# okian/kofft

Measured on AMD Instinct MI355X. Metric: batched 4096-pt c32 FFT throughput, GPoints/s (achieved HBM GB/s: roofline.achieved), higher is better.
Workload: dtype f32

## Files before the change

include/kofft_hip.h:

```cpp
#ifndef KOFFT_HIP_H
#define KOFFT_HIP_H

#include <stddef.h>

#ifdef __cplusplus
extern "C" {
#endif

#define KOFFT_OK 0
#define KOFFT_ERR_EMPTY_INPUT 1
#define KOFFT_ERR_NON_POWER_OF_TWO_NO_STD 2
#define KOFFT_ERR_MISMATCHED_LENGTHS 3
#define KOFFT_ERR_INVALID_STRIDE 4
#define KOFFT_ERR_INVALID_HOP_SIZE 5
#define KOFFT_ERR_INVALID_VALUE 6
#define KOFFT_ERR_HIP (-1)
#define KOFFT_ERR_UNSUPPORTED (-2)
#define KOFFT_ERR_NULL (-3)
#define KOFFT_ERR_ALLOC (-4)
#define KOFFT_ERR_RCCL (-5)

typedef struct kofft_hip_ctx kofft_hip_ctx;

const char *kofft_hip_strerror(int status);
// ... 58 lines not shown
int kofft_hip_rfft_f64_dev(kofft_hip_ctx *ctx, const double *d_in, double *d_out,
                           const double *d_window, size_t n, size_t batch);
int kofft_hip_irfft_f64(kofft_hip_ctx *ctx, const double *in, double *out, size_t n, size_t batch);
int kofft_hip_irfft_f64_dev(kofft_hip_ctx *ctx, const double *d_in, double *d_out, size_t n,
                            size_t batch);

int kofft_hip_dct2_f32(kofft_hip_ctx *ctx, const float *in, float *out, size_t n, size_t batch);
int kofft_hip_dct2_f32_dev(kofft_hip_ctx *ctx, const float *d_in, float *d_out, size_t n, size_t batch);
int kofft_hip_set_dct_fused(kofft_hip_ctx *ctx, int on);

int kofft_hip_hilbert_f32(kofft_hip_ctx *ctx, const float *in, float *out, size_t n, size_t batch);
int kofft_hip_hilbert_f32_dev(kofft_hip_ctx *ctx, const float *d_in, float *d_out, size_t n, size_t batch);
int kofft_hip_set_hilbert_fused(kofft_hip_ctx *ctx, int on);

int kofft_hip_cepstrum_f32(kofft_hip_ctx *ctx, const float *in, float *out, size_t n, size_t batch);
int kofft_hip_cepstrum_f32_dev(kofft_hip_ctx *ctx, const float *d_in, float *d_out, size_t n, size_t batch);
int kofft_hip_set_cepstrum_fused(kofft_hip_ctx *ctx, int on);

int kofft_hip_dct_direct_f32(kofft_hip_ctx *ctx, int type, const float *in, float *out, size_t n, size_t batch);
int kofft_hip_dct_direct_f32_dev(kofft_hip_ctx *ctx, int type, const float *d_in, float *d_out, size_t n, size_t batch);
int kofft_hip_dst_direct_f32(kofft_hip_ctx *ctx, int type, const float *in, float *out, size_t n, size_t batch);
int kofft_hip_dst_direct_f32_dev(kofft_hip_ctx *ctx, int type, const float *d_in, float *d_out, size_t n, size_t batch);
int kofft_hip_set_direct_tiled(kofft_hip_ctx *ctx, int on);
int kofft_hip_dct_direct_table_f32(int type, size_t n, float *C);
int kofft_hip_dst_direct_table_f32(int type, size_t n, float *C);
int kofft_hip_dst_planner_table_f32(int type, size_t n, float *out);
int kofft_hip_dst_planner_table_f64(int type, size_t n, double *out);

int kofft_hip_czt_f32(kofft_hip_ctx *ctx, const float *in, float *out, size_t n, size_t m, float wr, float wi, float ar, float ai,
                      size_t batch);
int kofft_hip_dev_czt_f32(kofft_hip_ctx *ctx, const float *d_in, float *d_out, size_t n, size_t m, float wr, float wi, float ar, float ai,
                          size_t batch);
int kofft_hip_goertzel_f32(kofft_hip_ctx *ctx, const float *in, float *out, size_t n, size_t batch, float sample_rate,
                           const float *target_freqs, size_t nfreq);
int kofft_hip_dev_goertzel_f32(kofft_hip_ctx *ctx, const float *d_in, float *d_out, size_t n, size_t batch, float sample_rate,
                               const float *target_freqs, size_t nfreq);
int kofft_hip_set_czt_route(kofft_hip_ctx *ctx, int mode);
int kofft_hip_czt_table_f32(size_t n, size_t m, float wr, float wi, float ar, float ai, float *C);
int kofft_hip_goertzel_coeff_f32(size_t n, float sample_rate, const float *target_freqs, size_t nfreq, float *coeff);

#define KOFFT_WAVELET_HAAR 0
#define KOFFT_WAVELET_DB2 1
#define KOFFT_WAVELET_DB4 2
#define KOFFT_WAVELET_SYM4 3
#define KOFFT_WAVELET_COIF1 4
int kofft_hip_dwt_f32(kofft_hip_ctx *ctx, int wavelet, const float *in, float *approx, float *detail, size_t len, size_t batch);
// ... 110 lines not shown
```

kofft_amd/_lib.py:

```python
from __future__ import annotations

import ctypes as C
import os
import re
from pathlib import Path

_PKG = Path(__file__).resolve().parent
LIB_PATH = _PKG / "lib" / "libkofft_hip.so"
HEADER_PATH = _PKG.parent / "include" / "kofft_hip.h"


class LibraryMissing(RuntimeError):
    pass


_c_f = C.POINTER(C.c_float)
_c_d = C.POINTER(C.c_double)
_sz = C.c_size_t
_ctx = C.c_void_p

SIGNATURES = {
    "kofft_hip_strerror": (C.c_char_p, [C.c_int]),
    "kofft_hip_last_error": (C.c_char_p, [_ctx]),
    "kofft_hip_version": (C.c_char_p, []),
# ... 33 lines not shown
    "kofft_hip_fft_c64_strided": (C.c_int, [_ctx, C.c_void_p, _sz, _sz, _sz, C.c_int]),
    "kofft_hip_rfft_f32": (C.c_int, [_ctx, C.c_void_p, C.c_void_p, C.c_void_p, _sz, _sz]),
    "kofft_hip_rfft_f32_dev": (C.c_int, [_ctx, C.c_void_p, C.c_void_p, C.c_void_p, _sz, _sz]),
    "kofft_hip_irfft_f32": (C.c_int, [_ctx, C.c_void_p, C.c_void_p, _sz, _sz]),
    "kofft_hip_irfft_f32_dev": (C.c_int, [_ctx, C.c_void_p, C.c_void_p, _sz, _sz]),
    "kofft_hip_rfft_f64": (C.c_int, [_ctx, C.c_void_p, C.c_void_p, C.c_void_p, _sz, _sz]),
    "kofft_hip_rfft_f64_dev": (C.c_int, [_ctx, C.c_void_p, C.c_void_p, C.c_void_p, _sz, _sz]),
    "kofft_hip_irfft_f64": (C.c_int, [_ctx, C.c_void_p, C.c_void_p, _sz, _sz]),
    "kofft_hip_irfft_f64_dev": (C.c_int, [_ctx, C.c_void_p, C.c_void_p, _sz, _sz]),
    "kofft_hip_dct2_f32": (C.c_int, [_ctx, C.c_void_p, C.c_void_p, _sz, _sz]),
    "kofft_hip_dct2_f32_dev": (C.c_int, [_ctx, C.c_void_p, C.c_void_p, _sz, _sz]),
    "kofft_hip_set_dct_fused": (C.c_int, [_ctx, C.c_int]),
    "kofft_hip_hilbert_f32": (C.c_int, [_ctx, C.c_void_p, C.c_void_p, _sz, _sz]),
    "kofft_hip_hilbert_f32_dev": (C.c_int, [_ctx, C.c_void_p, C.c_void_p, _sz, _sz]),
    "kofft_hip_set_hilbert_fused": (C.c_int, [_ctx, C.c_int]),
    "kofft_hip_cepstrum_f32": (C.c_int, [_ctx, C.c_void_p, C.c_void_p, _sz, _sz]),
    "kofft_hip_cepstrum_f32_dev": (C.c_int, [_ctx, C.c_void_p, C.c_void_p, _sz, _sz]),
    "kofft_hip_set_cepstrum_fused": (C.c_int, [_ctx, C.c_int]),
    "kofft_hip_dct_direct_f32": (C.c_int, [_ctx, C.c_int, C.c_void_p, C.c_void_p, _sz, _sz]),
    "kofft_hip_dct_direct_f32_dev": (C.c_int, [_ctx, C.c_int, C.c_void_p, C.c_void_p, _sz, _sz]),
    "kofft_hip_dst_direct_f32": (C.c_int, [_ctx, C.c_int, C.c_void_p, C.c_void_p, _sz, _sz]),
    "kofft_hip_dst_direct_f32_dev": (C.c_int, [_ctx, C.c_int, C.c_void_p, C.c_void_p, _sz, _sz]),
    "kofft_hip_set_direct_tiled": (C.c_int, [_ctx, C.c_int]),
    "kofft_hip_dct_direct_table_f32": (C.c_int, [C.c_int, _sz, C.c_void_p]),
    "kofft_hip_dst_direct_table_f32": (C.c_int, [C.c_int, _sz, C.c_void_p]),
    "kofft_hip_dst_planner_table_f32": (C.c_int, [C.c_int, _sz, C.c_void_p]),
    "kofft_hip_dst_planner_table_f64": (C.c_int, [C.c_int, _sz, C.c_void_p]),
    "kofft_hip_czt_f32": (C.c_int, [_ctx, C.c_void_p, C.c_void_p, _sz, _sz, C.c_float, C.c_float, C.c_float, C.c_float, _sz]),
    "kofft_hip_dev_czt_f32": (C.c_int, [_ctx, C.c_void_p, C.c_void_p, _sz, _sz, C.c_float, C.c_float, C.c_float, C.c_float, _sz]),
    "kofft_hip_goertzel_f32": (C.c_int, [_ctx, C.c_void_p, C.c_void_p, _sz, _sz, C.c_float, C.c_void_p, _sz]),
    "kofft_hip_dev_goertzel_f32": (C.c_int, [_ctx, C.c_void_p, C.c_void_p, _sz, _sz, C.c_float, C.c_void_p, _sz]),
    "kofft_hip_set_czt_route": (C.c_int, [_ctx, C.c_int]),
    "kofft_hip_czt_table_f32": (C.c_int, [_sz, _sz, C.c_float, C.c_float, C.c_float, C.c_float, C.c_void_p]),
    "kofft_hip_goertzel_coeff_f32": (C.c_int, [_sz, C.c_float, C.c_void_p, _sz, C.c_void_p]),
    "kofft_hip_dwt_f32": (C.c_int, [_ctx, C.c_int, C.c_void_p, C.c_void_p, C.c_void_p, _sz, _sz]),
    "kofft_hip_dwt_f32_dev": (C.c_int, [_ctx, C.c_int, C.c_void_p, C.c_void_p, C.c_void_p, _sz, _sz]),
    "kofft_hip_idwt_f32": (C.c_int, [_ctx, C.c_int, C.c_void_p, C.c_void_p, C.c_void_p, _sz, _sz]),
    "kofft_hip_idwt_f32_dev": (C.c_int, [_ctx, C.c_int, C.c_void_p, C.c_void_p, C.c_void_p, _sz, _sz]),
    "kofft_hip_dwt_multi_f32": (C.c_int, [_ctx, C.c_int, C.c_void_p, C.c_void_p, C.c_void_p, _sz, _sz, _sz]),
    "kofft_hip_dwt_multi_f32_dev": (C.c_int, [_ctx, C.c_int, C.c_void_p, C.c_void_p, C.c_void_p, _sz, _sz, _sz]),
    "kofft_hip_idwt_multi_f32": (C.c_int, [_ctx, C.c_int, C.c_void_p, C.c_void_p, C.c_void_p, C.c_void_p, _sz, _sz, _sz]),
    "kofft_hip_idwt_multi_f32_dev": (C.c_int, [_ctx, C.c_int, C.c_void_p, C.c_void_p, C.c_void_p, C.c_void_p, _sz, _sz, _sz]),
    "kofft_hip_set_wavelet_fused": (C.c_int, [_ctx, C.c_int]),
    "kofft_hip_dwt_multi_lengths": (C.c_int, [_sz, _sz, C.c_void_p]),
    "kofft_hip_wavelet_taps_f32": (C.c_int, [C.c_int, C.c_int, C.c_void_p, C.c_void_p]),
    "kofft_hip_stft_f32": (C.c_int, [_ctx, C.c_void_p, _sz, C.c_void_p, _sz, _sz, C.c_void_p, _sz]),
# ... 78 lines not shown
```

kofft_amd/api.py:

```python
from __future__ import annotations

import ctypes as C
import os
import enum
from typing import Optional, Sequence

import numpy as np

from . import _lib


class FftError(Exception):

    EmptyInput = 1
    NonPowerOfTwoNoStd = 2
    MismatchedLengths = 3
    InvalidStride = 4
    InvalidHopSize = 5
    InvalidValue = 6
    _names = {1: "EmptyInput", 2: "NonPowerOfTwoNoStd", 3: "MismatchedLengths", 4: "InvalidStride",
              5: "InvalidHopSize", 6: "InvalidValue"}

    def __init__(self, code: int):
        self.code = int(code)
# ... 495 lines not shown
        self._check(getattr(self._lib, f"kofft_hip_{family}_direct_f32")(self._ctx, int(type), _ptr(a), _ptr(out), a.shape[1], a.shape[0]))
        return out

    def dct_direct_batch(self, x: np.ndarray, type: int) -> np.ndarray:
        return self._direct_batch("dct", x, type)

    def dst_direct_batch(self, x: np.ndarray, type: int) -> np.ndarray:
        return self._direct_batch("dst", x, type)

    def _direct_dev(self, family: str, type: int, d_in: int, d_out: int, n: int, batch: int) -> None:
        if min(int(n), int(batch)) < 0:
            raise ValueError("n and batch are usize in the reference: they cannot be negative")
        self._check(getattr(self._lib, f"kofft_hip_{family}_direct_f32_dev")(self._ctx, int(type), C.c_void_p(d_in), C.c_void_p(d_out),
                                                                             int(n), int(batch)))

    def dct_direct_dev(self, type: int, d_in: int, d_out: int, n: int, batch: int) -> None:
        self._direct_dev("dct", type, d_in, d_out, n, batch)

    def dst_direct_dev(self, type: int, d_in: int, d_out: int, n: int, batch: int) -> None:
        self._direct_dev("dst", type, d_in, d_out, n, batch)

    def set_direct_tiled(self, on: bool) -> None:
        self._check(self._lib.kofft_hip_set_direct_tiled(self._ctx, int(bool(on))))

    def set_czt_route(self, mode: int) -> None:
        self._check(self._lib.kofft_hip_set_czt_route(self._ctx, int(mode)))

    def _spectral_in(self, x, what: str):
        if self.dtype != np.float32:
            raise TypeError(f"{what} is f32-only, like the reference ({what}.rs)")
        dev = hasattr(x, "data_ptr") and hasattr(x, "is_cuda")
        if dev:
            import torch

            if not x.is_cuda or x.dtype != torch.float32:
                raise TypeError(f"{what}: a torch input must be a float32 tensor on the device")
            a = x.contiguous()
        else:
            a = np.ascontiguousarray(x, np.float32)
        if a.ndim not in (1, 2):
            raise TypeError(f"{what} expects a 1-D signal or a 2-D [batch, n] array")
        return (a.reshape(1, -1) if a.ndim == 1 else a), a.ndim == 1, dev

    def czt(self, x, m: int, w, a):
        rows, one, dev = self._spectral_in(x, "czt")
        if int(m) < 0:
# ... 1019 lines not shown
```

kofft_amd/csrc/fft_persist.hip.h:

```cpp
#pragma once

#include "fft_wg.hip.h"

namespace kofft {

template <typename T, int L, int S0, int Q>
__device__ __forceinline__ void load_pass_twiddles(cpx<T> *twr, const int k, const cpx<T> *__restrict__ tw)
{
#pragma unroll
    for (int t = 0; t < Q; ++t) {
#pragma unroll
        for (int h = 0; h < (1 << t); ++h) {
            const int idx = (k << (L - 1 - S0 - t)) + (bitrev(h, t) << (L - 1 - t));
            twr[(1 << t) - 1 + h] = tw[idx];
        }
    }
}

template <typename T, int Q>
__device__ __forceinline__ void reg_pass_r(cpx<T> *v, const cpx<T> *twr)
{
#pragma unroll
    for (int t = 0; t < Q; ++t) {
        const int pos = Q - 1 - t;
// ... 73 lines not shown
}

template <bool WAVE>
__device__ __forceinline__ void exchange_sync()
{
    if constexpr (WAVE) {
        __builtin_amdgcn_fence(__ATOMIC_RELEASE, "wavefront");
        __builtin_amdgcn_wave_barrier();
        __builtin_amdgcn_fence(__ATOMIC_ACQUIRE, "wavefront");
    } else {
        __syncthreads();
    }
}

template <class CFG, class = void>
struct persist_depth { static constexpr int value = 1; };
template <class CFG>
struct persist_depth<CFG, decltype((void)CFG::DEPTH)> { static constexpr int value = CFG::DEPTH; };

template <class CFG, class = void>
struct persist_tw_global { static constexpr bool value = false; };
template <class CFG>
struct persist_tw_global<CFG, decltype((void)CFG::kTwGlobal)> { static constexpr bool value = CFG::kTwGlobal; };

template <typename T, int L, int RL, int EPI, class IO, class CFG>
struct PersistState {
    static constexpr int R = 1 << RL;
    static constexpr int NP = (L + RL - 1) / RL;
    static constexpr bool TWG = persist_tw_global<CFG>::value;
    static constexpr bool TW1_REG = !TWG && !(NP == 2 && CFG::kTwLastInLds);
    static constexpr bool TW2_REG = !TWG && NP >= 3 && !(CFG::kTwLastInLds && NP == 3);
    static constexpr bool TW3_REG = !TWG && NP >= 4 && !CFG::kTwLastInLds;
    cpx<T> tw1[TW1_REG ? R - 1 : 1], tw2[TW2_REG ? R - 1 : 1], tw3[TW3_REG ? R - 1 : 1];
    typename IO::Inv inv[CFG::kInvInLds ? 1 : R];
    const typename IO::Inv *inv_lds;
    const cpx<T> *tw_lds;
    const cpx<T> *rt_lds;
    int g1, g2, g3, sc;
};

template <class IO, int TPT, bool PAIR = io_pairs_in_wave<IO>::value>
struct persist_raw {
    using type = typename IO::Raw;
    static constexpr int extra = 0;
    static constexpr bool pair = false, pair_lds = false;
};
template <class IO, int TPT>
struct persist_raw<IO, TPT, true> {
    using type = typename IO::RawPair;
    static constexpr int extra = 1;
    static constexpr bool pair = TPT <= 64, pair_lds = TPT > 64;
};

struct NoAcc {};
template <class IO, bool HAS = io_has_acc<IO>::value>
struct persist_acc { using type = NoAcc; };
template <class IO>
struct persist_acc<IO, true> { using type = typename IO::Acc; };

#ifndef KOFFT_TWG_TOP_PART
#define KOFFT_TWG_TOP_PART -1
#endif
__host__ __device__ constexpr bool persist_twg_top_part(int L) { return KOFFT_TWG_TOP_PART < 0 ? L <= 12 : KOFFT_TWG_TOP_PART != 0; }
struct NoPrefetchParts {
    __device__ __forceinline__ void operator()(int) const {}
};
template <typename T, int L, int RL, int EPI, class CFG, class IO, class Parts = NoPrefetchParts>
__device__ __forceinline__ void persist_transform(const typename persist_raw<IO, ((1 << L) >> RL)>::type *raw,
                                                  const PersistState<T, L, RL, EPI, IO, CFG> &st,
                                                  const IO &io, const cpx<T> *__restrict__ tw, cpx<T> *buf0, cpx<T> *buf1,
                                                  const size_t xf0, const int cnt, const int sub, const int tau,
                                                  typename persist_acc<IO>::type &acc, const Parts &part = Parts{})
{
    constexpr int NBUF = CFG::NBUF;
    constexpr int N = 1 << L;
    constexpr int R = 1 << RL;
    constexpr int TPT = N / R;
    constexpr int NP = (L + RL - 1) / RL;
    constexpr bool WAVE = (TPT <= 64);
    const size_t xf = xf0 + sub;
    const bool active = sub < cnt;
    using LastG = PassGeom<L, RL, NP - 1>;
    using FirstG = PassGeom<L, RL, 0>;

    cpx<T> cur[R];
    constexpr int GRP = TPT >= 64 ? 1 : 64 / TPT;
    if constexpr (persist_raw<IO, TPT>::pair) {
        static_assert(CFG::kInvInLds, "paired input: the table entries come from the LDS copy");
        io.template finish_pairs<R, TPT>(raw, tau, cur, [&](int u) { return (st.inv_lds + tau)[FirstG::in_index(0, u)]; });
    } else if constexpr (persist_raw<IO, TPT>::pair_lds) {
        static_assert(CFG::kInvInLds && NBUF == 1 && !WAVE, "paired input through the exchange buffer");
        exchange_sync<WAVE>();
#pragma unroll
        for (int u = 0; u < R; ++u) buf0[tau + u * TPT] = raw[u];
        if (tau == 0) buf0[N] = raw[R];
// ... 26 lines not shown
    if (NBUF == 1) exchange_sync<WAVE>();
    persist_lds_scatter<T, L, RL, 0>(cur, buf0, st.sc);
    exchange_sync<WAVE>();
    persist_lds_gather<T, L, RL, 1>(cur, buf0, st.g1);
    using St = PersistState<T, L, RL, EPI, IO, CFG>;
    int tau_tw = tau;
    if constexpr (St::TWG) asm volatile("" : "+v"(tau_tw));
    auto pass_tw_global = [&](auto pass) {
        constexpr int P = decltype(pass)::value;
        using Gp = PassGeom<L, RL, P>;
        cpx<T> twr[Gp::G * ((1 << Gp::Q) - 1)];
        persist_load_tw<T, L, RL, P>(twr, tau_tw, tw);
        __builtin_amdgcn_sched_barrier(0);
        part(P - (persist_twg_top_part(L) ? 0 : 1));
        __builtin_amdgcn_sched_barrier(0);
        persist_compute<T, L, RL, P>(cur, twr);
    };
    if constexpr (St::TWG) pass_tw_global(std::integral_constant<int, 1>{});
    else if constexpr (NP == 2 && CFG::kTwLastInLds) wg_compute<T, L, RL, 1>(cur, io, st.tw_lds, xf, tau);
    else persist_compute<T, L, RL, 1>(cur, st.tw1);
    if constexpr (NP >= 3) {
        if (NBUF == 1) exchange_sync<WAVE>();
        persist_lds_scatter<T, L, RL, 1>(cur, buf1, st.sc);
        exchange_sync<WAVE>();
        persist_lds_gather<T, L, RL, 2>(cur, buf1, st.g2);
        if constexpr (St::TWG) pass_tw_global(std::integral_constant<int, 2>{});
        else if constexpr (NP == 3 && CFG::kTwLastInLds) wg_compute<T, L, RL, 2>(cur, io, st.tw_lds, xf, tau);
        else persist_compute<T, L, RL, 2>(cur, st.tw2);
    }
    if constexpr (NP == 4) {
        exchange_sync<WAVE>();
        persist_lds_scatter<T, L, RL, 2>(cur, buf0, st.sc);
        exchange_sync<WAVE>();
        persist_lds_gather<T, L, RL, 3>(cur, buf0, st.g3);
        if constexpr (St::TWG) pass_tw_global(std::integral_constant<int, 3>{});
        else if constexpr (CFG::kTwLastInLds) wg_compute<T, L, RL, 3>(cur, io, st.tw_lds, xf, tau);
        else persist_compute<T, L, RL, 3>(cur, st.tw3);
    }

    if constexpr (EPI == EPI_RFFT) {
        static_assert(L <= 12 || !CFG::kInvInLds, "rfft epilogue: a staged window does not fit next to an 8192-point exchange buffer and the post-pass table");
        cpx<T> *ybuf = (NP == 3) ? buf0 : buf1;
        if (NBUF == 1) exchange_sync<WAVE>();
        {
            cpx<T> *p = ybuf + tau;
#pragma unroll
            for (int u = 0; u < R; ++u) p[LastG::out_index(0, u)] = cur[u];
// ... 126 lines not shown
            for (int i = tid; i < N; i += BLOCK) inv_lds[i] = io.invariant(i);
        } else {
#pragma unroll
            for (int u = 0; u < R; ++u) st.inv[u] = io.invariant(FirstG::in_index(0, u) + tau);
        }
        if constexpr (EPI == EPI_RFFT) {
            for (int i = tid; i < N; i += BLOCK) rt_lds[i] = io.rtab[i];
        }
        if constexpr (CFG::kTwLastInLds) {
            for (int i = tid; i < N / 2; i += BLOCK) tw_lds[i] = tw[i];
        }
        st.inv_lds = inv_lds;
        st.rt_lds = rt_lds;
        st.tw_lds = tw_lds;
        if constexpr (CFG::kInvInLds || CFG::kTwLastInLds || EPI == EPI_RFFT) __syncthreads();
    }
    st.g1 = lds_pad(PassGeom<L, RL, 1>::in_index(tau, 0));
    st.g2 = (NP >= 3) ? lds_pad(PassGeom<L, RL, (NP >= 3 ? 2 : 1)>::in_index(tau, 0)) : 0;
    st.g3 = (NP == 4) ? lds_pad(PassGeom<L, RL, NP - 1>::in_index(tau, 0)) : 0;
    st.sc = lds_pad(tau);

    const size_t step = (size_t)gridDim.x * XPB;
    size_t base = (size_t)blockIdx.x * XPB;
    if (base >= batch) return;

    constexpr int DEPTH = persist_depth<CFG>::value;
    static_assert(DEPTH == 1 || DEPTH == 2, "prefetch distance");
    Raw ra[RS], rb[RS];
    const int in_lane_bytes = tau * IO::kRawBytes;
    const int in_row_off = (G == 1) ? 0 : sub * (int)io.in_slot_bytes();
    auto group_cnt = [&](size_t b) -> int {
        const size_t first = b + wslot;
        return first >= batch ? 0 : (batch - first < (size_t)G ? (int)(batch - first) : G);
    };
    auto issue = [&](Raw *dst, const size_t b) {
        const rsrc_t d = io.in_desc_n(b + wslot, group_cnt(b));
        if constexpr (RawSel::pair || RawSel::pair_lds) {
#pragma unroll
            for (int u = 0; u < R; ++u) dst[u] = io.fetch_pair_d(d, in_lane_bytes, FirstG::in_index(0, u), in_row_off);
            dst[R] = io.fetch_last_d(d, in_row_off);
        } else {
#pragma unroll
            for (int u = 0; u < R; ++u) dst[u] = io.fetch_d(d, in_lane_bytes, FirstG::in_index(0, u), in_row_off);
        }
    };
    issue(ra, base);
    typename persist_acc<IO>::type acc{};
    if constexpr (io_has_acc<IO>::value) acc = io.acc_init();
    auto finish = [&]() {
        if constexpr (io_has_acc<IO>::value) io.acc_finish(acc);
    };

    if constexpr (DEPTH == 1 && St::TWG && !(RawSel::pair || RawSel::pair_lds)) {
        constexpr bool TOP = persist_twg_top_part(L);
        constexpr int PARTS = TOP ? NP : NP - 1;
#define KOFFT_PERSIST_STEP_PARTS(CUR, NXT, LEAVE)                                                                    \
    {                                                                                                                \
        const size_t nbase = base + step;                                                                            \
        const bool more = nbase < batch;                                                      \
        const rsrc_t nd = io.in_desc_n(nbase + wslot, group_cnt(nbase));                                             \
        auto part = [&](const int i) {                                                                               \
            _Pragma("unroll") for (int u = 0; u < R; ++u)                                                            \
                if (u * PARTS / R == i) NXT[u] = io.fetch_d(nd, in_lane_bytes, FirstG::in_index(0, u), in_row_off);  \
        };                                                                                                           \
        if constexpr (TOP) {                                                                                         \
            part(0);                                                                                                 \
            __builtin_amdgcn_sched_barrier(0);                                                                       \
        }                                                                                                            \
        persist_transform<T, L, RL, EPI, CFG>(CUR, st, io, tw, buf0, buf1, base + wslot, group_cnt(base), sub, tau, acc, part); \
        if (!more) LEAVE;                                                                                            \
        base = nbase;                                                                                                \
    }
        KOFFT_PERSIST_STEP_PARTS(ra, rb, { finish(); return; })
        for (;;) {
            KOFFT_PERSIST_STEP_PARTS(rb, ra, break)
            KOFFT_PERSIST_STEP_PARTS(ra, rb, break)
        }
        finish();
#undef KOFFT_PERSIST_STEP_PARTS
    } else if constexpr (DEPTH == 1) {
#define KOFFT_PERSIST_STEP(CUR, NXT, LEAVE)                                                                          \
    {                                                                                                                \
        const size_t nbase = base + step;                                                                            \
        const bool more = nbase < batch;                                                      \
        issue(NXT, nbase);                                                                                           \
        __builtin_amdgcn_sched_barrier(0);                           \
        persist_transform<T, L, RL, EPI, CFG>(CUR, st, io, tw, buf0, buf1, base + wslot, group_cnt(base), sub, tau, acc); \
        if (!more) LEAVE;                                                                                            \
        base = nbase;                                                                                                \
    }
        KOFFT_PERSIST_STEP(ra, rb, { finish(); return; })
        for (;;) {
            KOFFT_PERSIST_STEP(rb, ra, break)
            KOFFT_PERSIST_STEP(ra, rb, break)
        }
        finish();
#undef KOFFT_PERSIST_STEP
    } else {
        Raw rc[RS];
        issue(rb, base + step);
#define KOFFT_PERSIST_STEP2(CUR, FAR, LEAVE)                                                                         \
    {                                                                                                                \
        const size_t nbase = base + step;                                                                            \
        const bool more = nbase < batch;                                                      \
        issue(FAR, nbase + step);                                                                                    \
        __builtin_amdgcn_sched_barrier(0);                                                                           \
        persist_transform<T, L, RL, EPI, CFG>(CUR, st, io, tw, buf0, buf1, base + wslot, group_cnt(base), sub, tau, acc); \
        if (!more) LEAVE;                                                                                            \
        base = nbase;                                                                                                \
    }
        KOFFT_PERSIST_STEP2(ra, rc, { finish(); return; })
        for (;;) {
            KOFFT_PERSIST_STEP2(rb, ra, break)
            KOFFT_PERSIST_STEP2(rc, rb, break)
            KOFFT_PERSIST_STEP2(ra, rc, break)
        }
        finish();
#undef KOFFT_PERSIST_STEP2
    }
}


}
```

kofft_amd/csrc/host_common.hip.h:

```cpp
#pragma once

#include "../../include/kofft_hip.h"

#include <hip/hip_runtime.h>

#include <atomic>
#include <cstdio>
#include <cstdlib>
#include <cstring>
#include <map>
#include <new>
#include <string>
#include <utility>
#include <vector>

#include "fft_big.hip.h"
#include "fft_persist.hip.h"
#include "fft_istft.hip.h"
#include "fft_regfile.hip.h"
#include "fft_split_wide.hip.h"
#include "fft_wg.hip.h"
#include "tables.h"

#define KOFFT_BIG_PROBE_MAX 8
struct kofft_spectral_slot {
    std::vector<unsigned> key;
    void *d_small = nullptr;
    void *d_table = nullptr;
};
constexpr size_t kSpectralSlots = 4;
struct kofft_hip_ctx {
    int device = 0;
    hipStream_t own_stream = nullptr;
    hipStream_t stream = nullptr;
    hipEvent_t order_event = nullptr;
    int num_cus = 256;
    bool use_persist = true;
    bool istft_fused = true;
    bool dct_fused = true;
    bool hilbert_fused = true;
    bool planar_fused = true;
    bool cepstrum_fused = true;
    bool direct_tiled = true;
    int wavelet_fused = 1;
    int czt_route = 0;
    bool blue_persist = true;
    int persist_grid_pct = 0;
    bool big_two_only = false;
    int big_three_min = 22;
    bool small32 = true;
    bool big_first11 = true;
    bool big_mid_group = true;
    int big_first_larger = -1;
    bool big_narrow = true;
    int big_narrow_per_cu = 1;
    bool big_persist = true;
    size_t big_persist_min_units = 32;
    int big_first_persist = -1;
    int big_mid_nt = -1;
    bool blue_fused = true;
    bool blue_one_kernel = true;
    bool nd_transpose = true;
    bool nd_fused = true;
    bool nd_two_pass = true;
    int nd_transpose_min = 4096;
    bool zero_copy = true;
    bool host_pipeline = true;
    int host_chunks = 0;
    bool rfft14_wide = true;
    bool rfft13_persist = true;
// ... 190 lines not shown
    hipLaunchKernelGGL(kern, dim3((unsigned)blocks), dim3(BLOCK), lds, ctx->stream, io, tw, batch);
    KOFFT_HIP_TRY(ctx, hipGetLastError());
    return KOFFT_OK;
}

template <int L, class IO> struct PersistCfg;
template <class IO> struct PersistCfgBase {
    static constexpr int NBUF = 1, RL = 4;
    static constexpr bool kInvInLds = IO::kInvInLds, kTwLastInLds = false;
};
template <class IO> struct PersistCfg<13, IO> : PersistCfgBase<IO> { static constexpr int BLOCK = 512, MINW = 2, WG_PER_CU = 1; };
template <bool INV> struct PersistCfg<13, ComplexIO<double, INV>> {
    static constexpr int BLOCK = 512, NBUF = 1, RL = 4, MINW = 2, WG_PER_CU = 1;
    static constexpr bool kInvInLds = false, kTwLastInLds = false, kTwGlobal = true;
};
template <bool INV> struct PersistCfg<12, ComplexIO<double, INV>> {
    static constexpr int BLOCK = 256, NBUF = 1, RL = 4, MINW = 2, WG_PER_CU = 2;
    static constexpr bool kInvInLds = false, kTwLastInLds = false, kTwGlobal = true;
};
#ifndef KOFFT_C12_DEPTH
#define KOFFT_C12_DEPTH 1
#endif
template <class IO> struct PersistCfg<12, IO> : PersistCfgBase<IO> { static constexpr int BLOCK = 256, MINW = 2, WG_PER_CU = 2, DEPTH = KOFFT_C12_DEPTH; };
template <class IO> struct PersistCfg<11, IO> : PersistCfgBase<IO> { static constexpr int BLOCK = 256, MINW = 2, WG_PER_CU = 2; };
template <class IO> struct PersistCfg<10, IO> : PersistCfgBase<IO> {
    static constexpr int BLOCK = 256, MINW = IO::kLeanRegisters ? 3 : 2, WG_PER_CU = MINW;
};
#ifndef KOFFT_RFFT10_DEPTH
#define KOFFT_RFFT10_DEPTH 2
#endif
template <> struct PersistCfg<10, RfftIO<float>> : PersistCfgBase<RfftIO<float>> {
    static constexpr int BLOCK = 256, MINW = 2, WG_PER_CU = 2, DEPTH = KOFFT_RFFT10_DEPTH;
};
#ifndef KOFFT_STFT10_DEPTH
#define KOFFT_STFT10_DEPTH 1
#endif
template <> struct PersistCfg<10, StftIO> : PersistCfgBase<StftIO> {
    static constexpr int BLOCK = 256, MINW = 2, WG_PER_CU = 2, DEPTH = KOFFT_STFT10_DEPTH;
};
template <> struct PersistCfg<10, StftMagIO> {
    static constexpr int BLOCK = 256, NBUF = 1, RL = 4, MINW = 3, WG_PER_CU = 3, DEPTH = KOFFT_STFT10_DEPTH;
    static constexpr bool kInvInLds = true, kTwLastInLds = false;
};
#ifndef KOFFT_IRFFT10_WG
#define KOFFT_IRFFT10_WG 2
#endif
// ... 52 lines not shown
    static constexpr int BLOCK = 256, NBUF = 1, RL = 3, MINW = 4, WG_PER_CU = 4;
    static constexpr bool kInvInLds = IO::kInvInLds, kTwLastInLds = false;
};
template <class IO> struct PersistCfg<9, IO> {
    static constexpr int BLOCK = 256, NBUF = 1, RL = 3, MINW = 4, WG_PER_CU = 4;
    static constexpr bool kInvInLds = IO::kInvInLds, kTwLastInLds = false;
};

template <int L, class IO> struct PersistGrid {
    static int wg_per_cu(int base, size_t) { return base; }
};
#ifndef KOFFT_RFFT6_WG
#define KOFFT_RFFT6_WG 3
#endif
template <> struct PersistGrid<6, RfftIO<float>> { static int wg_per_cu(int, size_t) { return KOFFT_RFFT6_WG; } };
template <> struct PersistGrid<7, RfftIO<float>> { static int wg_per_cu(int base, size_t) { return base / 2; } };
template <> struct PersistGrid<8, RfftIO<float>> { static int wg_per_cu(int base, size_t) { return base / 2; } };
template <> struct PersistGrid<9, RfftIO<float>> { static int wg_per_cu(int base, size_t) { return base / 2; } };
template <> struct PersistGrid<10, RfftIO<float>> {
    static int wg_per_cu(int base, size_t input_bytes) { return input_bytes > (size_t(1) << 30) ? base / 2 : base; }
};

template <typename T, int L, int EPI, class IO>
int launch_persist(kofft_hip_ctx *ctx, const IO &io, const cpx<T> *tw, size_t batch)
{
    using Cfg = PersistCfg<L, IO>;
    constexpr int RL = Cfg::RL;
    constexpr int XPB = Cfg::BLOCK / ((1 << L) >> RL);
    constexpr size_t lds = (size_t)XPB * Cfg::NBUF * persist_slot_elems(L) * sizeof(cpx<T>) +
                           (Cfg::kInvInLds ? (size_t)(1 << L) * sizeof(typename IO::Inv) : 0) +
                           (EPI == EPI_RFFT ? (size_t)(1 << L) * sizeof(cpx<T>) : 0) +
                           (Cfg::kTwLastInLds ? (size_t)(1 << L) / 2 * sizeof(cpx<T>) : 0);
    static_assert(lds * Cfg::WG_PER_CU <= 160 * 1024, "LDS budget");
    auto kern = fft_persist_kernel<T, L, RL, EPI, IO, Cfg>;
    {
        static std::atomic<unsigned long long> attr_done{0};
        const int arc = set_dyn_lds_once(ctx, attr_done, reinterpret_cast<const void *>(kern), lds);
        if (arc) return arc;
    }
    size_t blocks = (size_t)ctx->num_cus * PersistGrid<L, IO>::wg_per_cu(Cfg::WG_PER_CU, batch * sizeof(cpx<T>) << L);
    if (ctx->persist_grid_pct > 0) blocks = blocks * (size_t)ctx->persist_grid_pct / 100;
    if (blocks < 1) blocks = 1;
    const size_t need = (batch + XPB - 1) / XPB;
    if (blocks > need) blocks = need;
    hipLaunchKernelGGL(kern, dim3((unsigned)blocks), dim3(Cfg::BLOCK), lds, ctx->stream, io, tw, batch);
    KOFFT_HIP_TRY(ctx, hipGetLastError());
    return KOFFT_OK;
}

template <typename T, int LA, int LB, class IO>
int launch_split(kofft_hip_ctx *ctx, const IO &io, const cpx<T> *tw, size_t batch)
{
    using Gm = SplitGeom<LA, LB>;
    constexpr size_t lds = 2 * (size_t)Gm::N * sizeof(cpx<T>) + 16;
    static_assert(lds <= 160 * 1024, "LDS budget");
    auto kern = fft_split_persist_kernel<T, LA, LB, IO>;
    {
        static std::atomic<unsigned long long> attr_done{0};
        const int arc = set_dyn_lds_once(ctx, attr_done, reinterpret_cast<const void *>(kern), lds);
        if (arc) return arc;
    }
    size_t blocks = (size_t)ctx->num_cus;
    if (ctx->persist_grid_pct > 0) blocks = blocks * (size_t)ctx->persist_grid_pct / 100;
    if (blocks < 1) blocks = 1;
    if (blocks > batch) blocks = batch;
    hipLaunchKernelGGL(kern, dim3((unsigned)blocks), dim3(Gm::TPT), lds, ctx->stream, io, tw, batch);
    KOFFT_HIP_TRY(ctx, hipGetLastError());
    return KOFFT_OK;
// ... 292 lines not shown
```

kofft_amd/csrc/k_complex_f32.hip:

```cpp
#include "complex_impl.hip.h"

namespace kofft {
namespace host {
extern template int fft_big_dev<float, false>(kofft_hip_ctx *, const float *, float *, size_t, size_t);
extern template int fft_big_dev<float, true>(kofft_hip_ctx *, const float *, float *, size_t, size_t);
extern template int fft_bluestein_dev<float, false>(kofft_hip_ctx *, const float *, float *, size_t, size_t);
extern template int fft_bluestein_dev<float, true>(kofft_hip_ctx *, const float *, float *, size_t, size_t);
template int fft_dev<float>(kofft_hip_ctx *, const float *, float *, size_t, size_t, int);
template int fft_radix4_dev<float>(kofft_hip_ctx *, const float *, float *, size_t, size_t, int);
}
}

#if defined(KOFFT_RF_STAMPS)
extern "C" int kofft_hip_exp_rf_stamps_f32(void *out, size_t bytes)
{
    return hipMemcpyFromSymbol(out, HIP_SYMBOL(kofft::g_rf_stamps), bytes) == hipSuccess ? 0 : -1;
}
#endif
```

kofft_amd/csrc/kofft_hip.hip:

```cpp
#include "host_common.hip.h"
#include "host_layout.h"

#include <algorithm>
#include <condition_variable>
#include <mutex>
#include <thread>

using namespace kofft;
using namespace kofft::host;

namespace {

template <class Up, class Run, class Down>
int pipeline_chunks(kofft_hip_ctx *ctx, size_t nchunks, Up up, Run run, Down down)
{
    hipStream_t s_in = nullptr, s_out = nullptr;
    std::vector<hipEvent_t> uploaded(nchunks, nullptr), done(nchunks, nullptr);
    auto cleanup = [&]() {
        for (size_t c = 0; c < nchunks; ++c) {
            if (uploaded[c]) (void)hipEventDestroy(uploaded[c]);
            if (done[c]) (void)hipEventDestroy(done[c]);
        }
        if (s_in) (void)hipStreamDestroy(s_in);
        if (s_out) (void)hipStreamDestroy(s_out);
// ... 509 lines not shown
    if (const char *e = getenv("KOFFT_HIP_BLUESTEIN_FUSED")) ctx->blue_fused = !(e[0] == '0');
    if (const char *e = getenv("KOFFT_HIP_BLUESTEIN_ONE")) ctx->blue_one_kernel = !(e[0] == '0');
    if (const char *e = getenv("KOFFT_HIP_BIG_NARROW")) ctx->big_narrow = !(e[0] == '0');
    if (const char *e = getenv("KOFFT_HIP_BIG_FIRST11")) ctx->big_first11 = !(e[0] == '0');
    if (const char *e = getenv("KOFFT_HIP_ND_TWO_PASS")) ctx->nd_two_pass = !(e[0] == '0');
    if (const char *e = getenv("KOFFT_HIP_ND_FUSED")) ctx->nd_fused = !(e[0] == '0');
    if (const char *e = getenv("KOFFT_HIP_BIG_ROW_PAIRS")) ctx->big_row_pairs = !(e[0] == '0');
    if (const char *e = getenv("KOFFT_HIP_BIG_BLOCKED")) ctx->big_blocked = !(e[0] == '0');
    if (const char *e = getenv("KOFFT_HIP_BIG_PROBE")) ctx->big_probe = atoi(e);
    if (const char *e = getenv("KOFFT_HIP_BIG_CHUNK_MB")) {
        const long mb = atol(e);
        if (mb > 0) ctx->big_chunk_bytes = (size_t)mb << 20;
    }
    {
        hipDeviceProp_t prop;
        if (hipGetDeviceProperties(&prop, device) == hipSuccess && prop.multiProcessorCount > 0)
            ctx->num_cus = prop.multiProcessorCount;
    }
    if (hipStreamCreateWithFlags(&ctx->own_stream, hipStreamNonBlocking) != hipSuccess) {
        delete ctx;
        return KOFFT_ERR_HIP;
    }
    ctx->stream = ctx->own_stream;
    *out = ctx;
    return KOFFT_OK;
}

int kofft_hip_destroy(kofft_hip_ctx *ctx)
{
    if (!ctx) return KOFFT_ERR_NULL;
    (void)hipSetDevice(ctx->device);
    (void)hipStreamSynchronize(ctx->stream);
    for (auto &kv : ctx->tables) (void)hipFree(kv.second);
    spectral_drop(ctx);
    drop_host_buffers(ctx);
    if (ctx->big_tmp && !ctx->big_tmp_external) (void)hipFree(ctx->big_tmp);
    if (ctx->blue_tmp) (void)hipFree(ctx->blue_tmp);
    if (ctx->real_tmp) (void)hipFree(ctx->real_tmp);
    if (ctx->rows_tmp) (void)hipFree(ctx->rows_tmp);
    if (ctx->order_event) (void)hipEventDestroy(ctx->order_event);
    if (ctx->own_stream) (void)hipStreamDestroy(ctx->own_stream);
    delete ctx;
    return KOFFT_OK;
}

int kofft_hip_set_stream(kofft_hip_ctx *ctx, void *hip_stream)
{
    if (!ctx) return KOFFT_ERR_NULL;
    hipStream_t next = hip_stream ? static_cast<hipStream_t>(hip_stream) : ctx->own_stream;
    if (next == ctx->stream) return KOFFT_OK;
    KOFFT_HIP_TRY(ctx, hipSetDevice(ctx->device));
    if (!ctx->order_event) KOFFT_HIP_TRY(ctx, hipEventCreateWithFlags(&ctx->order_event, hipEventDisableTiming));
    KOFFT_HIP_TRY(ctx, hipEventRecord(ctx->order_event, ctx->stream));
    KOFFT_HIP_TRY(ctx, hipStreamWaitEvent(next, ctx->order_event, 0));
    ctx->stream = next;
    return KOFFT_OK;
}

int kofft_hip_synchronize(kofft_hip_ctx *ctx)
{
    if (!ctx) return KOFFT_ERR_NULL;
    KOFFT_HIP_TRY(ctx, hipStreamSynchronize(ctx->stream));
// ... 254 lines not shown
{
    return hilbert_dev(ctx, d_in, d_out, n, batch);
}
int kofft_hip_set_cepstrum_fused(kofft_hip_ctx *ctx, int on)
{
    if (!ctx) return KOFFT_ERR_NULL;
    ctx->cepstrum_fused = on != 0;
    return KOFFT_OK;
}
int kofft_hip_cepstrum_f32(kofft_hip_ctx *ctx, const float *in, float *out, size_t n, size_t batch)
{
    return cepstrum_host(ctx, in, out, n, batch);
}
int kofft_hip_cepstrum_f32_dev(kofft_hip_ctx *ctx, const float *d_in, float *d_out, size_t n, size_t batch)
{
    return cepstrum_dev(ctx, d_in, d_out, n, batch);
}
int kofft_hip_set_direct_tiled(kofft_hip_ctx *ctx, int on)
{
    if (!ctx) return KOFFT_ERR_NULL;
    ctx->direct_tiled = on != 0;
    return KOFFT_OK;
}
int kofft_hip_set_wavelet_fused(kofft_hip_ctx *ctx, int on)
{
    if (!ctx) return KOFFT_ERR_NULL;
    if (on < 0 || on > 2) return KOFFT_ERR_INVALID_VALUE;
    ctx->wavelet_fused = on;
    return KOFFT_OK;
}
int kofft_hip_dwt_f32(kofft_hip_ctx *ctx, int wavelet, const float *in, float *approx, float *detail, size_t len, size_t batch)
{
    return dwt_host(ctx, wavelet, in, approx, detail, len, batch);
}
int kofft_hip_dwt_f32_dev(kofft_hip_ctx *ctx, int wavelet, const float *d_in, float *d_approx, float *d_detail, size_t len, size_t batch)
{
    return dwt_dev(ctx, wavelet, d_in, d_approx, d_detail, len, batch);
}
int kofft_hip_idwt_f32(kofft_hip_ctx *ctx, int wavelet, const float *approx, const float *detail, float *out, size_t n, size_t batch)
{
    return idwt_host(ctx, wavelet, approx, detail, out, n, batch);
}
int kofft_hip_idwt_f32_dev(kofft_hip_ctx *ctx, int wavelet, const float *d_approx, const float *d_detail, float *d_out, size_t n, size_t batch)
{
    return idwt_dev(ctx, wavelet, d_approx, d_detail, d_out, n, batch);
}
// ... 268 lines not shown
```

Measured before the change: 356.2.

## Add dynamic atomic work-claiming tail for 4096-point complex f32 persistent FFT

For the 4096-point complex f32 persistent kernel, blocks walk the first part of the batch in a static grid stride, then claim the remaining rows (by default the last quarter) through a global atomic counter. The next ticket is fetched during the transform and handed to the block through LDS at an existing barrier. The aim is to even out tail imbalance between workgroups. The cost is atomic traffic, a reset protocol run by the last block to leave, an extra device allocation per context, and optional timestamp instrumentation.

```diff
diff --git a/include/kofft_hip.h b/include/kofft_hip.h
--- a/include/kofft_hip.h
+++ b/include/kofft_hip.h
@@ -104,6 +104,7 @@
 int kofft_hip_dst_direct_f32(kofft_hip_ctx *ctx, int type, const float *in, float *out, size_t n, size_t batch);
 int kofft_hip_dst_direct_f32_dev(kofft_hip_ctx *ctx, int type, const float *d_in, float *d_out, size_t n, size_t batch);
 int kofft_hip_set_direct_tiled(kofft_hip_ctx *ctx, int on);
+int kofft_hip_set_persist_claim_pct(kofft_hip_ctx *ctx, int pct);
 int kofft_hip_dct_direct_table_f32(int type, size_t n, float *C);
 int kofft_hip_dst_direct_table_f32(int type, size_t n, float *C);
 int kofft_hip_dst_planner_table_f32(int type, size_t n, float *out);
diff --git a/kofft_amd/_lib.py b/kofft_amd/_lib.py
--- a/kofft_amd/_lib.py
+++ b/kofft_amd/_lib.py
@@ -79,6 +79,7 @@
     "kofft_hip_dst_direct_f32": (C.c_int, [_ctx, C.c_int, C.c_void_p, C.c_void_p, _sz, _sz]),
     "kofft_hip_dst_direct_f32_dev": (C.c_int, [_ctx, C.c_int, C.c_void_p, C.c_void_p, _sz, _sz]),
     "kofft_hip_set_direct_tiled": (C.c_int, [_ctx, C.c_int]),
+    "kofft_hip_set_persist_claim_pct": (C.c_int, [_ctx, C.c_int]),
     "kofft_hip_dct_direct_table_f32": (C.c_int, [C.c_int, _sz, C.c_void_p]),
     "kofft_hip_dst_direct_table_f32": (C.c_int, [C.c_int, _sz, C.c_void_p]),
     "kofft_hip_dst_planner_table_f32": (C.c_int, [C.c_int, _sz, C.c_void_p]),
diff --git a/kofft_amd/api.py b/kofft_amd/api.py
--- a/kofft_amd/api.py
+++ b/kofft_amd/api.py
@@ -541,6 +541,9 @@
 
     def set_direct_tiled(self, on: bool) -> None:
         self._check(self._lib.kofft_hip_set_direct_tiled(self._ctx, int(bool(on))))
+
+    def set_persist_claim_pct(self, pct: int) -> None:
+        self._check(self._lib.kofft_hip_set_persist_claim_pct(self._ctx, int(pct)))
 
     def set_czt_route(self, mode: int) -> None:
         self._check(self._lib.kofft_hip_set_czt_route(self._ctx, int(mode)))
diff --git a/kofft_amd/csrc/fft_persist.hip.h b/kofft_amd/csrc/fft_persist.hip.h
--- a/kofft_amd/csrc/fft_persist.hip.h
+++ b/kofft_amd/csrc/fft_persist.hip.h
@@ -119,6 +119,41 @@
 struct persist_tw_global { static constexpr bool value = false; };
 template <class CFG>
 struct persist_tw_global<CFG, decltype((void)CFG::kTwGlobal)> { static constexpr bool value = CFG::kTwGlobal; };
+
+template <class CFG, class = void>
+struct persist_claim { static constexpr bool value = false; };
+template <class CFG>
+struct persist_claim<CFG, decltype((void)CFG::kClaim)> { static constexpr bool value = CFG::kClaim; };
+
+struct PersistClaim {
+    unsigned *counters;
+    size_t split;
+};
+template <class IO>
+struct PersistClaimIO : IO {
+    PersistClaim claim;
+};
+struct NoXchg {
+    __device__ __forceinline__ void put() const {}
+    __device__ __forceinline__ void get() const {}
+};
+
+#ifdef KOFFT_PERSIST_STAMPS
+constexpr int kPersistStampWgs = 4096, kPersistStampWords = 16;
+static __device__ unsigned long long g_persist_stamps[kPersistStampWgs * kPersistStampWords];
+__device__ __forceinline__ unsigned long long persist_stamp()
+{
+    unsigned long long t;
+    asm volatile("s_memtime %0\n\ts_waitcnt lgkmcnt(0)" : "=s"(t)::"memory");
+    return t;
+}
+__device__ __forceinline__ unsigned long long persist_stamp_real()
+{
+    unsigned long long t;
+    asm volatile("s_memrealtime %0\n\ts_waitcnt lgkmcnt(0)" : "=s"(t)::"memory");
+    return t;
+}
+#endif
 
 template <typename T, int L, int RL, int EPI, class IO, class CFG>
 struct PersistState {
@@ -162,12 +197,12 @@
 struct NoPrefetchParts {
     __device__ __forceinline__ void operator()(int) const {}
 };
-template <typename T, int L, int RL, int EPI, class CFG, class IO, class Parts = NoPrefetchParts>
+template <typename T, int L, int RL, int EPI, class CFG, class IO, class Parts = NoPrefetchParts, class Xchg = NoXchg>
 __device__ __forceinline__ void persist_transform(const typename persist_raw<IO, ((1 << L) >> RL)>::type *raw,
                                                   const PersistState<T, L, RL, EPI, IO, CFG> &st,
                                                   const IO &io, const cpx<T> *__restrict__ tw, cpx<T> *buf0, cpx<T> *buf1,
                                                   const size_t xf0, const int cnt, const int sub, const int tau,
-                                                  typename persist_acc<IO>::type &acc, const Parts &part = Parts{})
+                                                  typename persist_acc<IO>::type &acc, const Parts &part = Parts{}, const Xchg &xchg = Xchg{})
 {
     constexpr int NBUF = CFG::NBUF;
     constexpr int N = 1 << L;
@@ -240,7 +275,9 @@
     if constexpr (NP >= 3) {
         if (NBUF == 1) exchange_sync<WAVE>();
         persist_lds_scatter<T, L, RL, 1>(cur, buf1, st.sc);
+        xchg.put();
         exchange_sync<WAVE>();
+        xchg.get();
         persist_lds_gather<T, L, RL, 2>(cur, buf1, st.g2);
         if constexpr (St::TWG) pass_tw_global(std::integral_constant<int, 2>{});
         else if constexpr (NP == 3 && CFG::kTwLastInLds) wg_compute<T, L, RL, 2>(cur, io, st.tw_lds, xf, tau);
@@ -413,7 +450,57 @@
 
     const size_t step = (size_t)gridDim.x * XPB;
     size_t base = (size_t)blockIdx.x * XPB;
-    if (base >= batch) return;
+    constexpr bool CLAIMS = persist_claim<CFG>::value;
+#ifdef KOFFT_PERSIST_STAMPS
+    const unsigned long long stamp_entry = persist_stamp(), stamp_entry_real = persist_stamp_real();
+    unsigned long long stamp_landed = 0, stamp_landed_real = 0, stamp_rows = 0;
+#define KOFFT_PERSIST_STAMP_LANDED()                                                                                  \
+    {                                                                                                                 \
+        asm volatile("s_waitcnt vmcnt(%0)" ::"n"(RS) : "memory");     \
+        stamp_landed = persist_stamp();                                                                               \
+        stamp_landed_real = persist_stamp_real();                                                                     \
+        __builtin_amdgcn_sched_barrier(0);                                                                            \
+    }
+#define KOFFT_PERSIST_STAMP_ROW() ++stamp_rows;
+#else
+#define KOFFT_PERSIST_STAMP_LANDED()
+#define KOFFT_PERSIST_STAMP_ROW()
+#endif
+    [[maybe_unused]] size_t nbase = 0;
+    [[maybe_unused]] unsigned long long *claim_word = nullptr;
+    if constexpr (CLAIMS) {
+        static_assert(NP == 3 && NBUF == 1 && !WAVE && G == 1 && persist_depth<CFG>::value == 1 && !persist_tw_global<CFG>::value &&
+                          !(RawSel::pair || RawSel::pair_lds) && !CFG::kInvInLds && !CFG::kTwLastInLds && EPI != EPI_RFFT,
+                      "claim hand-out: block-synchronised three-pass transforms, one row ahead, nothing else in LDS");
+        claim_word = reinterpret_cast<unsigned long long *>(smem_raw + (size_t)XPB * NBUF * persist_slot_elems(L) * sizeof(cpx<T>));
+        const bool first_walked = io.claim.split > 0;
+        const bool second_walked = first_walked && base + step < io.claim.split;
+        nbase = base + step;
+        if (!second_walked) {
+            if (tid == 0) {
+                size_t r0 = base, r1 = batch;
+                if (!first_walked) r0 = io.claim.split + (size_t)XPB * atomicAdd(io.claim.counters, 1u);
+                if (r0 < batch) r1 = io.claim.split + (size_t)XPB * atomicAdd(io.claim.counters, 1u);
+                claim_word[0] = r0;
+                claim_word[1] = r1;
+            }
+            __syncthreads();
+            base = claim_word[0];
+            nbase = claim_word[1];
+        }
+    }
+    [[maybe_unused]] auto claim_leave = [&]() {
+        if constexpr (CLAIMS) {
+            if (tid == 0 && atomicAdd(io.claim.counters + 1, 1u) == gridDim.x - 1) {
+                __hip_atomic_store(io.claim.counters, 0u, __ATOMIC_RELAXED, __HIP_MEMORY_SCOPE_AGENT);
+                __hip_atomic_store(io.claim.counters + 1, 0u, __ATOMIC_RELAXED, __HIP_MEMORY_SCOPE_AGENT);
+            }
+        }
+    };
+    if (base >= batch) {
+        if constexpr (CLAIMS) claim_leave();
+        return;
+    }
 
     constexpr int DEPTH = persist_depth<CFG>::value;
     static_assert(DEPTH == 1 || DEPTH == 2, "prefetch distance");
@@ -440,9 +527,72 @@
     if constexpr (io_has_acc<IO>::value) acc = io.acc_init();
     auto finish = [&]() {
         if constexpr (io_has_acc<IO>::value) io.acc_finish(acc);
+        if constexpr (CLAIMS) claim_leave();
+#ifdef KOFFT_PERSIST_STAMPS
+        if (tid == 0 && blockIdx.x < kPersistStampWgs) {
+            unsigned long long *rec = g_persist_stamps + (size_t)blockIdx.x * kPersistStampWords;
+            rec[0] = stamp_entry;
+            rec[1] = stamp_landed;
+            rec[2] = persist_stamp();
+            rec[3] = stamp_entry_real;
+            rec[4] = stamp_landed_real;
+            rec[5] = persist_stamp_real();
+            rec[6] = stamp_rows;
+            rec[7] = __builtin_amdgcn_s_getreg((31 << 11) | 4);
+            rec[8] = __builtin_amdgcn_s_getreg((31 << 11) | 20);
+            rec[9] = gridDim.x;
+            rec[10] = 1;
+        }
+#endif
     };
 
-    if constexpr (DEPTH == 1 && St::TWG && !(RawSel::pair || RawSel::pair_lds)) {
+    if constexpr (CLAIMS) {
+        unsigned claim_index = 0;
+        asm volatile("" : "+v"(claim_index));
+        unsigned *const claim_next = io.claim.counters + claim_index;
+        struct ClaimXchg {
+            unsigned long long *word;
+            size_t split;
+            const unsigned *ticket;
+            size_t *claimed;
+            bool writer;
+            __device__ __forceinline__ void put() const
+            {
+                if (writer) *word = split + (size_t)XPB * *ticket;
+            }
+            __device__ __forceinline__ void get() const { *claimed = *word; }
+        };
+#define KOFFT_PERSIST_STEP_CLAIM(CUR, NXT, LEAVE)                                                                    \
+    {                                                                                                                \
+        const bool more = nbase < batch;                                                      \
+        const bool walked = nbase + step < io.claim.split;                                    \
+        const bool claims = more && !walked && tid == 0;                                                             \
+        unsigned ticket;  \
+        size_t claimed = batch;                                                                                      \
+        if (claims) ticket = atomicAdd(claim_next, 1u);                                                              \
+        __builtin_amdgcn_sched_barrier(0);                                   \
+        issue(NXT, nbase);                                                                                           \
+        __builtin_amdgcn_sched_barrier(0);                           \
+        KOFFT_PERSIST_STEP_STAMP                                                                                     \
+        const ClaimXchg xchg{claim_word, io.claim.split, &ticket, &claimed, claims};                                 \
+        persist_transform<T, L, RL, EPI, CFG>(CUR, st, io, tw, buf0, buf1, base + wslot, group_cnt(base), sub, tau, acc, NoPrefetchParts{}, xchg); \
+        KOFFT_PERSIST_STAMP_ROW()                                                                                    \
+        if (!more) LEAVE;                                                                                            \
+        base = nbase;                                                                                                \
+        nbase = walked ? nbase + step : (size_t)claimed;                 \
+    }
+#define KOFFT_PERSIST_STEP_STAMP KOFFT_PERSIST_STAMP_LANDED()
+        KOFFT_PERSIST_STEP_CLAIM(ra, rb, { finish(); return; })
+#undef KOFFT_PERSIST_STEP_STAMP
+#define KOFFT_PERSIST_STEP_STAMP
+        for (;;) {
+            KOFFT_PERSIST_STEP_CLAIM(rb, ra, break)
+            KOFFT_PERSIST_STEP_CLAIM(ra, rb, break)
+        }
+#undef KOFFT_PERSIST_STEP_STAMP
+        finish();
+#undef KOFFT_PERSIST_STEP_CLAIM
+    } else if constexpr (DEPTH == 1 && St::TWG && !(RawSel::pair || RawSel::pair_lds)) {
         constexpr bool TOP = persist_twg_top_part(L);
         constexpr int PARTS = TOP ? NP : NP - 1;
 #define KOFFT_PERSIST_STEP_PARTS(CUR, NXT, LEAVE)                                                                    \
@@ -476,15 +626,21 @@
         const bool more = nbase < batch;                                                      \
         issue(NXT, nbase);                                                                                           \
         __builtin_amdgcn_sched_barrier(0);                           \
+        KOFFT_PERSIST_STEP_STAMP                                                                                                     \
         persist_transform<T, L, RL, EPI, CFG>(CUR, st, io, tw, buf0, buf1, base + wslot, group_cnt(base), sub, tau, acc); \
+        KOFFT_PERSIST_STAMP_ROW()                                                                                    \
         if (!more) LEAVE;                                                                                            \
         base = nbase;                                                                                                \
     }
+#define KOFFT_PERSIST_STEP_STAMP KOFFT_PERSIST_STAMP_LANDED()
         KOFFT_PERSIST_STEP(ra, rb, { finish(); return; })
+#undef KOFFT_PERSIST_STEP_STAMP
+#define KOFFT_PERSIST_STEP_STAMP
         for (;;) {
             KOFFT_PERSIST_STEP(rb, ra, break)
             KOFFT_PERSIST_STEP(ra, rb, break)
         }
+#undef KOFFT_PERSIST_STEP_STAMP
         finish();
 #undef KOFFT_PERSIST_STEP
     } else {
@@ -511,5 +667,7 @@
     }
 }
 
-
-}
+#undef KOFFT_PERSIST_STAMP_LANDED
+#undef KOFFT_PERSIST_STAMP_ROW
+
+}
diff --git a/kofft_amd/csrc/host_common.hip.h b/kofft_amd/csrc/host_common.hip.h
--- a/kofft_amd/csrc/host_common.hip.h
+++ b/kofft_amd/csrc/host_common.hip.h
@@ -46,6 +46,8 @@
     int czt_route = 0;
     bool blue_persist = true;
     int persist_grid_pct = 0;
+    int persist_claim_pct = -1;
+    unsigned *persist_claim_counters = nullptr;
     bool big_two_only = false;
     int big_three_min = 22;
     bool small32 = true;
@@ -282,6 +284,16 @@
 #define KOFFT_C12_DEPTH 1
 #endif
 template <class IO> struct PersistCfg<12, IO> : PersistCfgBase<IO> { static constexpr int BLOCK = 256, MINW = 2, WG_PER_CU = 2, DEPTH = KOFFT_C12_DEPTH; };
+#ifndef KOFFT_C12_CLAIM
+#define KOFFT_C12_CLAIM true
+#endif
+#ifndef KOFFT_C12_CLAIM_PCT
+#define KOFFT_C12_CLAIM_PCT 25
+#endif
+template <bool INV> struct PersistCfg<12, ComplexIO<float, INV>> : PersistCfgBase<ComplexIO<float, INV>> {
+    static constexpr int BLOCK = 256, MINW = 2, WG_PER_CU = 2, DEPTH = KOFFT_C12_DEPTH, kClaimPct = KOFFT_C12_CLAIM_PCT;
+    static constexpr bool kClaim = KOFFT_C12_CLAIM;
+};
 template <class IO> struct PersistCfg<11, IO> : PersistCfgBase<IO> { static constexpr int BLOCK = 256, MINW = 2, WG_PER_CU = 2; };
 template <class IO> struct PersistCfg<10, IO> : PersistCfgBase<IO> {
     static constexpr int BLOCK = 256, MINW = IO::kLeanRegisters ? 3 : 2, WG_PER_CU = MINW;
@@ -380,9 +392,13 @@
 };
 
 template <typename T, int L, int EPI, class IO>
+int launch_persist_claim(kofft_hip_ctx *ctx, const IO &io, const cpx<T> *tw, size_t batch);
+template <typename T, int L, int EPI, class IO>
 int launch_persist(kofft_hip_ctx *ctx, const IO &io, const cpx<T> *tw, size_t batch)
 {
     using Cfg = PersistCfg<L, IO>;
+    if constexpr (persist_claim<Cfg>::value) return launch_persist_claim<T, L, EPI>(ctx, io, tw, batch);
+    else {
     constexpr int RL = Cfg::RL;
     constexpr int XPB = Cfg::BLOCK / ((1 << L) >> RL);
     constexpr size_t lds = (size_t)XPB * Cfg::NBUF * persist_slot_elems(L) * sizeof(cpx<T>) +
@@ -402,6 +418,40 @@
     const size_t need = (batch + XPB - 1) / XPB;
     if (blocks > need) blocks = need;
     hipLaunchKernelGGL(kern, dim3((unsigned)blocks), dim3(Cfg::BLOCK), lds, ctx->stream, io, tw, batch);
+    KOFFT_HIP_TRY(ctx, hipGetLastError());
+    return KOFFT_OK;
+    }
+}
+
+template <typename T, int L, int EPI, class IO>
+int launch_persist_claim(kofft_hip_ctx *ctx, const IO &io, const cpx<T> *tw, size_t batch)
+{
+    using Cfg = PersistCfg<L, IO>;
+    constexpr int RL = Cfg::RL;
+    constexpr int XPB = Cfg::BLOCK / ((1 << L) >> RL);
+    constexpr size_t lds = (size_t)XPB * Cfg::NBUF * persist_slot_elems(L) * sizeof(cpx<T>) + 16;
+    static_assert(lds * Cfg::WG_PER_CU <= 160 * 1024, "LDS budget");
+    if (!ctx->persist_claim_counters) {
+        ctx->last_error = "the context has no claim counters";
+        return KOFFT_ERR_ALLOC;
+    }
+    using KIO = PersistClaimIO<IO>;
+    auto kern = fft_persist_kernel<T, L, RL, EPI, KIO, Cfg>;
+    {
+        static std::atomic<unsigned long long> attr_done{0};
+        const int arc = set_dyn_lds_once(ctx, attr_done, reinterpret_cast<const void *>(kern), lds);
+        if (arc) return arc;
+    }
+    size_t blocks = (size_t)ctx->num_cus * PersistGrid<L, IO>::wg_per_cu(Cfg::WG_PER_CU, batch * sizeof(cpx<T>) << L);
+    if (ctx->persist_grid_pct > 0) blocks = blocks * (size_t)ctx->persist_grid_pct / 100;
+    if (blocks < 1) blocks = 1;
+    const size_t need = (batch + XPB - 1) / XPB;
+    if (blocks > need) blocks = need;
+    const size_t stride = blocks * XPB;
+    const size_t pct = ctx->persist_claim_pct < 0 ? (size_t)Cfg::kClaimPct : (ctx->persist_claim_pct > 100 ? 100 : (size_t)ctx->persist_claim_pct);
+    const size_t claimed = batch / 100 * pct + batch % 100 * pct / 100;
+    const KIO kio{io, PersistClaim{ctx->persist_claim_counters, (batch - claimed) / stride * stride}};
+    hipLaunchKernelGGL(kern, dim3((unsigned)blocks), dim3(Cfg::BLOCK), lds, ctx->stream, kio, tw, batch);
     KOFFT_HIP_TRY(ctx, hipGetLastError());
     return KOFFT_OK;
 }
diff --git a/kofft_amd/csrc/k_complex_f32.hip b/kofft_amd/csrc/k_complex_f32.hip
--- a/kofft_amd/csrc/k_complex_f32.hip
+++ b/kofft_amd/csrc/k_complex_f32.hip
@@ -17,3 +17,14 @@
     return hipMemcpyFromSymbol(out, HIP_SYMBOL(kofft::g_rf_stamps), bytes) == hipSuccess ? 0 : -1;
 }
 #endif
+#if defined(KOFFT_PERSIST_STAMPS)
+extern "C" int kofft_hip_exp_persist_stamps_f32(void *out, size_t bytes)
+{
+    return hipMemcpyFromSymbol(out, HIP_SYMBOL(kofft::g_persist_stamps), bytes) == hipSuccess ? 0 : -1;
+}
+extern "C" int kofft_hip_exp_persist_stamps_clear_f32(void)
+{
+    static const unsigned long long zeros[kofft::kPersistStampWgs * kofft::kPersistStampWords] = {};
+    return hipMemcpyToSymbol(HIP_SYMBOL(kofft::g_persist_stamps), zeros, sizeof(zeros)) == hipSuccess ? 0 : -1;
+}
+#endif
diff --git a/kofft_amd/csrc/kofft_hip.hip b/kofft_amd/csrc/kofft_hip.hip
--- a/kofft_amd/csrc/kofft_hip.hip
+++ b/kofft_amd/csrc/kofft_hip.hip
@@ -555,6 +555,13 @@
         return KOFFT_ERR_HIP;
     }
     ctx->stream = ctx->own_stream;
+    if (hipMalloc(reinterpret_cast<void **>(&ctx->persist_claim_counters), 64) != hipSuccess ||
+        hipMemsetAsync(ctx->persist_claim_counters, 0, 64, ctx->own_stream) != hipSuccess) {
+        if (ctx->persist_claim_counters) (void)hipFree(ctx->persist_claim_counters);
+        (void)hipStreamDestroy(ctx->own_stream);
+        delete ctx;
+        return KOFFT_ERR_ALLOC;
+    }
     *out = ctx;
     return KOFFT_OK;
 }
@@ -571,6 +578,7 @@
     if (ctx->blue_tmp) (void)hipFree(ctx->blue_tmp);
     if (ctx->real_tmp) (void)hipFree(ctx->real_tmp);
     if (ctx->rows_tmp) (void)hipFree(ctx->rows_tmp);
+    if (ctx->persist_claim_counters) (void)hipFree(ctx->persist_claim_counters);
     if (ctx->order_event) (void)hipEventDestroy(ctx->order_event);
     if (ctx->own_stream) (void)hipStreamDestroy(ctx->own_stream);
     delete ctx;
@@ -871,6 +879,13 @@
     ctx->direct_tiled = on != 0;
     return KOFFT_OK;
 }
+int kofft_hip_set_persist_claim_pct(kofft_hip_ctx *ctx, int pct)
+{
+    if (!ctx) return KOFFT_ERR_NULL;
+    if (pct > 100) return KOFFT_ERR_INVALID_VALUE;
+    ctx->persist_claim_pct = pct < 0 ? -1 : pct;
+    return KOFFT_OK;
+}
 int kofft_hip_set_wavelet_fused(kofft_hip_ctx *ctx, int on)
 {
     if (!ctx) return KOFFT_ERR_NULL;
```

New measurement: 376.2 (median of 6 runs). 1.06x the previous value.
